# privefl/bigsnpr

Hardware: NVIDIA H100
Metric: genotypes/sec in bed_prodVec (higher is better)
Workload: dtype f64

## Files before the change

### bigsnpr_b200/csrc/bsg_pmv.cu

```cuda
#include <algorithm>
#include <math.h>
#include <stdio.h>
#include <stdlib.h>
#include <string.h>

#include <cub/device/device_scan.cuh>

#include "bsg_internal.cuh"
#include "bsg_pmv_shared.cuh"

namespace bsg {
namespace pmv {

constexpr int SEG = 128;
constexpr int CODES = 512;
constexpr int DIG = 4096;
constexpr int STAGES = 6;
constexpr int STAGE_BYTES = 2 * DIG;
constexpr int SMEM_BYTES = STAGES * STAGE_BYTES + 128;
constexpr int MAX_CHUNKS_PER_ITEM = 512;

struct Args {
  const uint8_t *P;
  int64_t stride;
// ... 532 lines not shown
  int ks_min = (a.nchunks + MAX_CHUNKS_PER_ITEM - 1) / MAX_CHUNKS_PER_ITEM;
  ks = std::min(ks, ks_max);
  ks = std::max(ks, ks_min);
  ks = std::max(ks, 1);
  a.chunks_per_split = (a.nchunks + ks - 1) / ks;
  a.ksplit = (a.nchunks + a.chunks_per_split - 1) / a.chunks_per_split;
  a.dig1 = dig1;
  a.dig2 = dig2;
  a.na_flags = na_flags;
  a.use_na = use_na;
  BSG_TRY(v->s_part.ensure((size_t)a.nlines_pad * 16 * sizeof(long long)));
  a.part = v->s_part.as<long long>();
  BSG_CUDA(cudaMemsetAsync(a.part, 0, (size_t)a.nlines_pad * 16 * sizeof(long long), s));
  const int mode = plane_hi ? 3 : (!use_na ? 0 : (dig2 ? 2 : 1));
  if (plane_hi && !dig2) return fail(BSG_ERR_ARG, "high-bit plane needs its own digits");
  void (*kern)(const Args) = nullptr;
#define PMV_PICK(CWv, Rv, Sv)                                                                   \
  if (var_cw == CWv && var_r == Rv && var_s == Sv)                                              \
    kern = mode == 0 ? k_pmv<0, CWv, Rv, Sv>                                                    \
                     : (mode == 1 ? k_pmv<1, CWv, Rv, Sv> : (mode == 2 ? k_pmv<2, CWv, Rv, Sv> : k_pmv<3, CWv, Rv, Sv>));
  PMV_PICK(11, 2, 0)
  PMV_PICK(11, 2, 1)
  PMV_PICK(11, 2, 2)
  PMV_PICK(11, 3, 0)
  PMV_PICK(11, 3, 1)
  PMV_PICK(15, 2, 1)
#undef PMV_PICK
  if (!kern) return fail(BSG_ERR_ARG, "unknown k_pmv variant");
  BSG_CUDA(cudaFuncSetAttribute(kern, cudaFuncAttributeMaxDynamicSharedMemorySize, SMEM_BYTES));
  int nsm = 132;
  cudaDeviceGetAttribute(&nsm, cudaDevAttrMultiProcessorCount, v->h->device);
  int nitems = ngroups * a.ksplit;
  int grid = std::min(nitems, nsm);
  if (g_timing) cudaEventRecord(g_ev0[g_ev_n % EV_POOL], s);
  kern<<<grid, (var_cw + 1) * 32, SMEM_BYTES, s>>>(a);
  if (g_timing) {
    cudaEventRecord(g_ev1[g_ev_n % EV_POOL], s);
    g_ev_n++;
  }
  count_launch();
  BSG_CUDA(cudaGetLastError());
  *out_args = a;
  return BSG_OK;
}

}

namespace pmvt {
using namespace pmv;
constexpr int TLINES = 32, TBYTES = 512, TWARPS = 8, TSTAGES = 6;
constexpr int WSTAGE_BYTES = TLINES * 64;
constexpr int TSMEM = TWARPS * TSTAGES * WSTAGE_BYTES;
constexpr int MAX_LINES_PER_ITEM = 1 << 16;

struct TArgs {
  const uint8_t *P;
  int64_t stride;
  const int *lines;
  int nlines;
  const uint8_t *dig;
  int lines_per_split, ksplit, nblocks, n;
  long long *part;
};

__device__ __forceinline__ void cp_async16(uint32_t dst, const void *src, int src_bytes) {
  asm volatile("cp.async.cg.shared.global [%0], [%1], 16, %2;" ::"r"(dst), "l"(src), "r"(src_bytes) : "memory");
}

template <int PLANE>
__global__ void __launch_bounds__(TWARPS * 32, 2) k_pmvT_lines(const TArgs a) {
  extern __shared__ __align__(128) uint8_t smem[];
  const int tid = threadIdx.x, warp = tid >> 5, lane = tid & 31, g = lane >> 2, q = lane & 3;
  const int blk = blockIdx.x % a.nblocks, ks = blockIdx.x / a.nblocks;
  const int64_t byte0 = (int64_t)blk * TBYTES + 64 * warp;
  const int l0 = ks * a.lines_per_split, l1 = min(a.nlines, l0 + a.lines_per_split);
  const int nsteps = (l1 - l0 + TLINES - 1) / TLINES;
  const uint32_t wbase = smem_u32(smem) + warp * (TSTAGES * WSTAGE_BYTES);

  const int lrow = lane >> 2, lch = lane & 3;
  const int64_t colb = (byte0 + 16 * lch < a.stride) ? byte0 + 16 * lch : 0;
  uint32_t dst_off[4];
#pragma unroll
  for (int i = 0; i < 4; i++) {
    const int row = 8 * i + lrow;
    const int hf = row >> 4, qq = (row >> 2) & 3, r = row & 3, sl = lch >> 1, hc = lch & 1;
    dst_off[i] = (uint32_t)((((((r * 2 + hf) * 2 + sl) * 4 + qq) * 8) + 4 * hc) * 4);
  }
  auto issue = [&](int step, int stage) {
    const uint32_t dst = wbase + stage * WSTAGE_BYTES;
#pragma unroll
    for (int i = 0; i < 4; i++) {
      const int t = min(l0 + step * TLINES + 8 * i + lrow, l1 - 1);
      const int phys = a.lines[t];
      cp_async16(dst + dst_off[i], a.P + colb + (int64_t)phys * a.stride, 16);
    }
  };

  int acc[4][4][4];
#pragma unroll
  for (int j = 0; j < 4; j++)
#pragma unroll
    for (int c = 0; c < 4; c++)
#pragma unroll
      for (int k = 0; k < 4; k++) acc[j][c][k] = 0;

#pragma unroll
  for (int st = 0; st < TSTAGES - 1; st++) {
    if (st < nsteps) issue(st, st);
    asm volatile("cp.async.commit_group;" ::: "memory");
  }
  const uint8_t *dg = a.dig + (int64_t)(l0 / TLINES) * 256 + g * 32 + 4 * q;
  uint32_t nb0 = 0, nb1 = 0;
  if (nsteps > 0) {
    nb0 = *reinterpret_cast<const uint32_t *>(dg);
    nb1 = *reinterpret_cast<const uint32_t *>(dg + 16);
  }
  const uint32_t rd_base = wbase + (uint32_t)((q * 8 + g) * 4);

  auto compute = [&](uint32_t st_base, uint32_t b0, uint32_t b1) {
    uint32_t W[2][2][4];
// ... 25 lines not shown
        wd = (wd >> 1) & 0x55555555u;
      }
      mma_u8s8(acc[j][0], wa & 0x03030303u, wb & 0x03030303u, wc2 & 0x03030303u, wd & 0x03030303u, b0, b1);
      mma_u8s8(acc[j][1], wa & 0x0C0C0C0Cu, wb & 0x0C0C0C0Cu, wc2 & 0x0C0C0C0Cu, wd & 0x0C0C0C0Cu, b0, b1);
      mma_u8s8(acc[j][2], wa & 0x30303030u, wb & 0x30303030u, wc2 & 0x30303030u, wd & 0x30303030u, b0, b1);
      mma_u8s8(acc[j][3], wa & 0xC0C0C0C0u, wb & 0xC0C0C0C0u, wc2 & 0xC0C0C0C0u, wd & 0xC0C0C0C0u, b0, b1);
    }
  };

  uint32_t rd_stage = 0, wr_stage = (TSTAGES - 1) * WSTAGE_BYTES;
  const uint8_t *dgn = dg + 256;
  for (int step = 0; step < nsteps; step++) {
    asm volatile("cp.async.wait_group %0;" ::"n"(TSTAGES - 2) : "memory");
    __syncwarp();
    {
      const int nxt = step + TSTAGES - 1;
      if (nxt < nsteps) issue(nxt, (int)(wr_stage / WSTAGE_BYTES));
      asm volatile("cp.async.commit_group;" ::: "memory");
    }
    const uint32_t b0 = nb0, b1 = nb1;
    if (step + 1 < nsteps) {
      nb0 = *reinterpret_cast<const uint32_t *>(dgn);
      nb1 = *reinterpret_cast<const uint32_t *>(dgn + 16);
      dgn += 256;
    }
    compute(rd_base + rd_stage, b0, b1);
    rd_stage = rd_stage + WSTAGE_BYTES == TSTAGES * WSTAGE_BYTES ? 0 : rd_stage + WSTAGE_BYTES;
    wr_stage = wr_stage + WSTAGE_BYTES == TSTAGES * WSTAGE_BYTES ? 0 : wr_stage + WSTAGE_BYTES;
  }
  asm volatile("cp.async.wait_group 0;" ::: "memory");
#pragma unroll
  for (int j = 0; j < 4; j++)
#pragma unroll
    for (int c = 0; c < 4; c++)
#pragma unroll
      for (int sl = 0; sl < 2; sl++) {
        const int64_t sample = 4 * (byte0 + 4 * (8 * sl + g) + j) + c;
        if (sample < a.n) {
          unsigned long long *dst = reinterpret_cast<unsigned long long *>(a.part) + sample * 16 + (PLANE ? 8 : 0) + 2 * q;
          long long v0 = acc[j][c][2 * sl], v1 = acc[j][c][2 * sl + 1];
          v0 >>= 2 * c;
          v1 >>= 2 * c;
          if (v0) atomicAdd(dst, (unsigned long long)v0);
          if (v1) atomicAdd(dst + 1, (unsigned long long)v1);
        }
      }
}

constexpr int TBOX = 32 * 128;
constexpr int TDIG_OFF = 4 * TBOX;
constexpr int TSTAGE_BYTES = 4 * TBOX + 1024;
constexpr int TCSTAGES = 6;
constexpr int TSMEM_TMA = TCSTAGES * TSTAGE_BYTES + 2 * TCSTAGES * 8 + 1024;


template <int PLANE>
__global__ void __launch_bounds__(TWARPS * 32, 2) k_pmvT(const __grid_constant__ CUtensorMap map, const TArgs a) {
  extern __shared__ __align__(128) uint8_t smem[];
  const int tid = threadIdx.x, warp = tid >> 5, lane = tid & 31, g = lane >> 2, q = lane & 3;
  const int blk = blockIdx.x % a.nblocks, ks = blockIdx.x / a.nblocks;
  const int l0 = ks * a.lines_per_split, l1 = min(a.nlines, l0 + a.lines_per_split);
  const int nsteps = (l1 - l0 + TLINES - 1) / TLINES;
  const uint32_t sbase = (smem_u32(smem) + 1023u) & ~1023u;
  const uint32_t bar_base = sbase + TCSTAGES * TSTAGE_BYTES;
  auto fill = [&](int step, int st) {
    const uint32_t full = bar_base + 8 * st, dst = sbase + st * TSTAGE_BYTES;
    const uint8_t *dg = a.dig + (int64_t)(l0 / TLINES + step) * 256;
    mbar_expect_tx(full, 4 * TBOX + 256);
#pragma unroll
    for (int j = 0; j < 4; j++) tma_load_2d(dst + j * TBOX, &map, full, blk * TBYTES + 128 * j, l0 + step * TLINES);
    bulk_g2s(dst + TDIG_OFF, dg, 128, full);
    bulk_g2s(dst + TDIG_OFF + 144, dg + 128, 128, full);
  };
  if (tid == 0) {
    for (int st = 0; st < TCSTAGES; st++) {
      mbar_init(bar_base + 8 * st, 1);
      mbar_init(bar_base + 8 * (TCSTAGES + st), TWARPS);
    }
    asm volatile("fence.mbarrier_init.release.cluster;" ::: "memory");
    for (int st = 0; st < min(TCSTAGES, nsteps); st++) fill(st, st);
  }
  __syncthreads();
  int stage = 0, pstage = 0;
  uint32_t phase = 0, pphase = 0;

  const int64_t byte0 = (int64_t)blk * TBYTES + 64 * warp;
  const int rsw = 2 * (q >> 1);
  const uint32_t chunk0 = (4 * (warp & 1) + (g >> 2)) ^ (4 * (q & 1) + rsw);
  const uint32_t rd_base = sbase + (warp >> 1) * TBOX + q * 512 + (rsw << 7) + chunk0 * 16 + 4 * (g & 3);
  const uint32_t dg_base = sbase + TDIG_OFF + g * 32 + 16 * (g >> 2) + 4 * q;
  const uint32_t sel_lo = rsw ? 0x1054u : 0x5410u, sel_hi = rsw ? 0x3276u : 0x7632u;

  int acc[4][4][4];
#pragma unroll
  for (int j = 0; j < 4; j++)
#pragma unroll
    for (int c = 0; c < 4; c++)
#pragma unroll
      for (int k = 0; k < 4; k++) acc[j][c][k] = 0;

  for (int step = 0; step < nsteps; step++) {
    const uint32_t full = bar_base + 8 * stage, empty = bar_base + 8 * (TCSTAGES + stage);
    const uint32_t so = stage * TSTAGE_BYTES;
    const int cstage = stage;
    const uint32_t cphase = phase;
    mbar_wait(full, phase);
    const uint32_t b0 = lds32(dg_base + so), b1 = lds32(dg_base + so + 16);
    uint32_t W[2][2][4];
#pragma unroll
    for (int sl = 0; sl < 2; sl++)
#pragma unroll
      for (int hf = 0; hf < 2; hf++) {
        const uint32_t ad = rd_base + so, hb = hf * (16 * 128);
        const uint32_t x0 = lds32((ad ^ TRD(0, sl)) + hb), x1 = lds32((ad ^ TRD(1, sl)) + hb);
        const uint32_t x2 = lds32((ad ^ TRD(2, sl)) + hb), x3 = lds32((ad ^ TRD(3, sl)) + hb);
        const uint32_t t0 = prmt(x0, x1, 0x5140), t1 = prmt(x2, x3, 0x5140);
        const uint32_t t2 = prmt(x0, x1, 0x7362), t3 = prmt(x2, x3, 0x7362);
        W[sl][hf][0] = prmt(t0, t1, sel_lo);
        W[sl][hf][1] = prmt(t0, t1, sel_hi);
        W[sl][hf][2] = prmt(t2, t3, sel_lo);
        W[sl][hf][3] = prmt(t2, t3, sel_hi);
      }
    __syncwarp();
    if (lane == 0) mbar_arrive(empty);
    if (++stage == TCSTAGES) {
      stage = 0;
      phase ^= 1;
    }
#pragma unroll
    for (int j = 0; j < 4; j++) {
      uint32_t wa = W[0][0][j], wb = W[1][0][j], wc2 = W[0][1][j], wd = W[1][1][j];
      if (PLANE == 1) {
        wa = wa & (wa >> 1) & 0x55555555u;
        wb = wb & (wb >> 1) & 0x55555555u;
        wc2 = wc2 & (wc2 >> 1) & 0x55555555u;
        wd = wd & (wd >> 1) & 0x55555555u;
      } else if (PLANE == 2) {
        wa = (wa >> 1) & 0x55555555u;
        wb = (wb >> 1) & 0x55555555u;
        wc2 = (wc2 >> 1) & 0x55555555u;
        wd = (wd >> 1) & 0x55555555u;
      }
      mma_u8s8(acc[j][0], wa & 0x03030303u, wb & 0x03030303u, wc2 & 0x03030303u, wd & 0x03030303u, b0, b1);
      mma_u8s8(acc[j][1], wa & 0x0C0C0C0Cu, wb & 0x0C0C0C0Cu, wc2 & 0x0C0C0C0Cu, wd & 0x0C0C0C0Cu, b0, b1);
      mma_u8s8(acc[j][2], wa & 0x30303030u, wb & 0x30303030u, wc2 & 0x30303030u, wd & 0x30303030u, b0, b1);
      mma_u8s8(acc[j][3], wa & 0xC0C0C0C0u, wb & 0xC0C0C0C0u, wc2 & 0xC0C0C0C0u, wd & 0xC0C0C0C0u, b0, b1);
    }
    if (tid == 0 && step >= 1 && step - 1 + TCSTAGES < nsteps) {
      mbar_wait(bar_base + 8 * (TCSTAGES + pstage), pphase);
      fill(step - 1 + TCSTAGES, pstage);
    }
    __syncwarp();
    pstage = cstage;
    pphase = cphase;
  }
#pragma unroll
  for (int j = 0; j < 4; j++)
#pragma unroll
    for (int c = 0; c < 4; c++)
#pragma unroll
      for (int sl = 0; sl < 2; sl++) {
        const int64_t sample = 4 * (byte0 + 4 * (8 * sl + g) + j) + c;
        if (sample < a.n) {
          unsigned long long *dst = reinterpret_cast<unsigned long long *>(a.part) + sample * 16 + (PLANE ? 8 : 0) + 2 * q;
          long long v0 = acc[j][c][2 * sl], v1 = acc[j][c][2 * sl + 1];
          v0 >>= 2 * c;
          v1 >>= 2 * c;
          if (v0) atomicAdd(dst, (unsigned long long)v0);
          if (v1) atomicAdd(dst + 1, (unsigned long long)v1);
        }
      }
}

constexpr int W2STAGE_BYTES = TLINES * 32;
constexpr int T2BYTES = TWARPS * 32;
constexpr int T2SMEM = TWARPS * TSTAGES * W2STAGE_BYTES;

template <int PL, bool LINES>
__global__ void __launch_bounds__(TWARPS * 32, 2) k_pmvT2(const TArgs a, const uint8_t *__restrict__ dig2) {
  extern __shared__ __align__(128) uint8_t smem[];
  const int tid = threadIdx.x, warp = tid >> 5, lane = tid & 31, g = lane >> 2, q = lane & 3;
  const int blk = blockIdx.x % a.nblocks, ks = blockIdx.x / a.nblocks;
  const int64_t byte0 = (int64_t)blk * T2BYTES + 32 * warp;
  const int l0 = ks * a.lines_per_split, l1 = min(a.nlines, l0 + a.lines_per_split);
  const int nsteps = (l1 - l0 + TLINES - 1) / TLINES;
  const uint32_t wbase = smem_u32(smem) + warp * (TSTAGES * W2STAGE_BYTES);
  const int lrow = lane >> 1, lch = lane & 1;
  const int64_t colb = (byte0 + 16 * lch < a.stride) ? byte0 + 16 * lch : 0;
  uint32_t dst_off[2];
#pragma unroll
  for (int i = 0; i < 2; i++) {
    const int row = 16 * i + lrow;
    const int hf = row >> 4, qq = (row >> 2) & 3, r = row & 3;
    dst_off[i] = (uint32_t)(((((r * 2 + hf) * 4 + qq) * 8) + 4 * lch) * 4);
  }
  const int full_steps = (l1 - l0) / TLINES;
  const int64_t stride16 = 16 * a.stride;
  auto issue = [&](int step, int stage) {
    const uint32_t dst = wbase + stage * W2STAGE_BYTES;
#pragma unroll
    for (int i = 0; i < 2; i++) {
      const int t = min(l0 + step * TLINES + 16 * i + lrow, l1 - 1);
      const int phys = LINES ? a.lines[t] : t;
      cp_async16(dst + dst_off[i], a.P + colb + (int64_t)phys * a.stride, 16);
    }
  };
  int acc[2][2][4][4];
#pragma unroll
  for (int p = 0; p < 2; p++)
#pragma unroll
    for (int u = 0; u < 2; u++)
#pragma unroll
      for (int c = 0; c < 4; c++)
#pragma unroll
        for (int k = 0; k < 4; k++) acc[p][u][c][k] = 0;
#pragma unroll
  for (int st = 0; st < TSTAGES - 1; st++) {
    if (st < nsteps) issue(st, st);
    asm volatile("cp.async.commit_group;" ::: "memory");
  }
  const int64_t doff = (int64_t)(l0 / TLINES) * 256 + g * 32 + 4 * q;
  const uint8_t *dg = a.dig + doff, *dp = dig2 + doff;
  uint32_t nb0 = 0, nb1 = 0, np0 = 0, np1 = 0;
  if (nsteps > 0) {
// ... 332 lines not shown
  using namespace pmvt;
  bsg_bed *h = v->h;
  const int n = h->n, nc = v->nc;
  const int nsteps = (nc + TLINES - 1) / TLINES;
  BSG_TRY(v->s_part.ensure((size_t)std::max(n, 1) * 16 * sizeof(long long)));
  long long *part = v->s_part.as<long long>();
  *part_out = part;
  BSG_CUDA(cudaMemsetAsync(part, 0, (size_t)n * 16 * sizeof(long long), s));
  if (nc == 0 || n == 0) return BSG_OK;
  TArgs a;
  a.P = h->A;
  a.stride = h->strideA;
  a.lines = v->d_col;
  a.nlines = nc;
  a.n = n;
  a.part = part;
  const int64_t nbytes = ((int64_t)n + 3) / 4;
  a.nblocks = (int)((nbytes + TBYTES - 1) / TBYTES);
  int nsm = 132;
  cudaDeviceGetAttribute(&nsm, cudaDevAttrMultiProcessorCount, h->device);
  static int waves = 0;
  if (!waves) {
    const char *ev = getenv("BSG_PMVT_WAVES");
    waves = ev ? std::max(1, std::min(64, atoi(ev))) : 4;
  }
  auto pick_ks = [&](int nblocks) {
    const int slots = 2 * nsm;
    const int lo = std::max(1, (nc + MAX_LINES_PER_ITEM - 1) / MAX_LINES_PER_ITEM);
    const int hi = std::max(lo, std::min(std::max(1, nsteps / 32), std::max(lo, (4 * waves * slots) / std::max(nblocks, 1))));
    static int force_ks = -1;
    if (force_ks < 0) {
      const char *ev = getenv("BSG_PMVT_KS");
      force_ks = ev ? std::max(0, atoi(ev)) : 0;
    }
    if (force_ks > 0) return std::max(lo, force_ks);
    int best = lo;
    double best_score = -1;
    for (int ks = lo; ks <= hi; ks++) {
      const double ctas = (double)nblocks * ks, nwav = ceil(ctas / slots);
      double score = ctas / (nwav * slots);
      const double lines = (double)nc / ks;
      score *= lines / (lines + 1000.0);
      if (nwav < waves) score *= 0.9 + 0.1 * nwav / waves;
      if (score > best_score + 1e-9) {
        best_score = score;
        best = ks;
      }
    }
    return best;
  };
  int ks = pick_ks(a.nblocks);
  a.lines_per_split = (int)round_up((nc + ks - 1) / ks, TLINES);
  a.ksplit = (nc + a.lines_per_split - 1) / a.lines_per_split;
  static unsigned attr_done = 0;
  if (!(attr_done >> (h->device & 31) & 1u)) {
    BSG_CUDA(cudaFuncSetAttribute(k_pmvT<0>, cudaFuncAttributeMaxDynamicSharedMemorySize, TSMEM_TMA));
    BSG_CUDA(cudaFuncSetAttribute(k_pmvT_lines<0>, cudaFuncAttributeMaxDynamicSharedMemorySize, TSMEM));
    BSG_CUDA(cudaFuncSetAttribute(k_pmvT2<1, false>, cudaFuncAttributeMaxDynamicSharedMemorySize, T2SMEM));
    BSG_CUDA(cudaFuncSetAttribute(k_pmvT2<1, true>, cudaFuncAttributeMaxDynamicSharedMemorySize, T2SMEM));
    BSG_CUDA(cudaFuncSetAttribute(k_pmvT2<2, false>, cudaFuncAttributeMaxDynamicSharedMemorySize, T2SMEM));
    BSG_CUDA(cudaFuncSetAttribute(k_pmvT2<2, true>, cudaFuncAttributeMaxDynamicSharedMemorySize, T2SMEM));
    attr_done |= 1u << (h->device & 31);
  }
  const int thr = TWARPS * 32;
  const bool lines = a.lines != nullptr;
  a.dig = dig_raw;
  if (g_timing) cudaEventRecord(g_ev0[g_ev_n % EV_POOL], s);
  if (!plane) {
    const int grid = a.nblocks * a.ksplit;
    if (lines) {
      k_pmvT_lines<0><<<grid, thr, TSMEM, s>>>(a);
    } else {
      CUtensorMap map;
      BSG_TRY(make_map(&map, a.P, nc, a.stride, TLINES));
      k_pmvT<0><<<grid, thr, TSMEM_TMA, s>>>(map, a);
    }
  } else {
    a.nblocks = (int)((nbytes + T2BYTES - 1) / T2BYTES);
    const int ks2 = pick_ks(a.nblocks);
    a.lines_per_split = (int)round_up((nc + ks2 - 1) / ks2, TLINES);
    a.ksplit = (nc + a.lines_per_split - 1) / a.lines_per_split;
    const int grid = a.nblocks * a.ksplit;
    if (plane == 1) {
      if (lines)
        k_pmvT2<1, true><<<grid, thr, T2SMEM, s>>>(a, dig_plane);
      else
        k_pmvT2<1, false><<<grid, thr, T2SMEM, s>>>(a, dig_plane);
    } else {
      if (lines)
        k_pmvT2<2, true><<<grid, thr, T2SMEM, s>>>(a, dig_plane);
      else
        k_pmvT2<2, false><<<grid, thr, T2SMEM, s>>>(a, dig_plane);
    }
  }
  if (g_timing) {
    cudaEventRecord(g_ev1[g_ev_n % EV_POOL], s);
    g_ev_n++;
  }
  count_launch();
  BSG_CUDA(cudaGetLastError());
  return BSG_OK;
}

static int prep_T(bsg_view *v, int mode, const double *x, const double *p1, const double *p2, int nv, const double *xb,
                  bool two, cudaStream_t s, long long *qna_full = nullptr, int na_second = 0) {
  using namespace pmv;
  using namespace pmvt;
  Scal *sc = v->s_scal.as<Scal>();
  const int nc = v->nc;
  const int nsteps = (nc + TLINES - 1) / TLINES;
  BSG_TRY(v->s_dig1.ensure((size_t)std::max(nsteps, 1) * 256));
  if (two) BSG_TRY(v->s_dig2.ensure((size_t)std::max(nsteps, 1) * 256));
  uint8_t *dig1 = v->s_dig1.as<uint8_t>(), *dig2 = two ? v->s_dig2.as<uint8_t>() : nullptr;
  BSG_CUDA(cudaMemsetAsync(sc, 0, nv * sizeof(Scal), s));
  k_prep1<<<SUMCZ_BLOCKS, 256, 0, s>>>(mode, x, p1, p2, nc, 0, sc);
  if (xb) k_prep1<<<SUMCZ_BLOCKS, 256, 0, s>>>(mode, xb, p1, p2, nc, 0, sc + 1);
  const int grid = launch_cap((int64_t)std::max(nsteps, 1) * TLINES, 256, 1184);
  if (nv == 1)
    k_quantT<1><<<grid, 256, 0, s>>>(mode, x, nullptr, p1, p2, nc, nsteps * TLINES, sc, dig1, dig2, v->d_col, qna_full,
                                     na_second);
  else
    k_quantT<2><<<grid, 256, 0, s>>>(mode, x, xb, p1, p2, nc, nsteps * TLINES, sc, dig1, dig2, nullptr, nullptr, 0);
  count_launch(xb ? 3 : 2);
  return BSG_OK;
}

static int prodvec_T(bsg_view *v, const double *x_dev, double *out_dev, cudaStream_t s, bsg_comm *comm) {
  using namespace pmv;
  bsg_bed *h = v->h;
  Scal *sc = v->s_scal.as<Scal>();
  const int n = h->n, nc = v->nc;
  const int mode = v->has_scaling ? 1 : 0;
  const bool lists = h->has_na && na_ell_ready(h);
  const bool two = v->has_scaling && h->has_na && !lists;
// ... 778 lines not shown
```

### bigsnpr_b200/csrc/bsg_pmv_shared.cuh

```cuda
#pragma once
#include <cuda.h>
#include <math.h>
#include <stdint.h>

namespace bsg {
namespace pmv {

constexpr int SUMCZ_BLOCKS = 128;

__device__ __forceinline__ uint32_t smem_u32(const void *p) { return (uint32_t)__cvta_generic_to_shared(p); }

__device__ __forceinline__ void mbar_init(uint32_t bar, uint32_t count) {
  asm volatile("mbarrier.init.shared::cta.b64 [%0], %1;" ::"r"(bar), "r"(count));
}
__device__ __forceinline__ void mbar_expect_tx(uint32_t bar, uint32_t bytes) {
  asm volatile("mbarrier.arrive.expect_tx.shared::cta.b64 _, [%0], %1;" ::"r"(bar), "r"(bytes) : "memory");
}
__device__ __forceinline__ void mbar_arrive(uint32_t bar) {
  asm volatile("mbarrier.arrive.shared::cta.b64 _, [%0];" ::"r"(bar) : "memory");
}
__device__ __forceinline__ void mbar_wait(uint32_t bar, uint32_t parity) {
  asm volatile(
      "{\n\t.reg .pred p;\n\t"
      "WAIT_%=:\n\t"
      "mbarrier.try_wait.parity.shared::cta.b64 p, [%0], %1;\n\t"
      "@p bra DONE_%=;\n\t"
      "bra WAIT_%=;\n\t"
      "DONE_%=:\n\t}" ::"r"(bar),
      "r"(parity)
      : "memory");
}
__device__ __forceinline__ void bulk_g2s(uint32_t dst, const void *src, uint32_t bytes, uint32_t bar) {
  asm volatile("cp.async.bulk.shared::cluster.global.mbarrier::complete_tx::bytes [%0], [%1], %2, [%3];" ::"r"(dst),
               "l"(src), "r"(bytes), "r"(bar)
               : "memory");
}
__device__ __forceinline__ void mma_u8s8(int (&d)[4], uint32_t a0, uint32_t a1, uint32_t a2, uint32_t a3,
                                         uint32_t b0, uint32_t b1) {
  asm volatile(
      "mma.sync.aligned.m16n8k32.row.col.s32.u8.s8.s32 {%0,%1,%2,%3}, {%4,%5,%6,%7}, {%8,%9}, {%0,%1,%2,%3};"
      : "+r"(d[0]), "+r"(d[1]), "+r"(d[2]), "+r"(d[3])
      : "r"(a0), "r"(a1), "r"(a2), "r"(a3), "r"(b0), "r"(b1));
}
__device__ __forceinline__ uint4 lds128(uint32_t addr) {
  uint4 v;
  asm volatile("ld.shared.v4.u32 {%0,%1,%2,%3}, [%4];" : "=r"(v.x), "=r"(v.y), "=r"(v.z), "=r"(v.w) : "r"(addr));
  return v;
}

__device__ __forceinline__ uint4 ldg_stream(const uint8_t *p) {
  uint4 v;
  asm volatile("ld.global.nc.L1::no_allocate.v4.u32 {%0,%1,%2,%3}, [%4];"
               : "=r"(v.x), "=r"(v.y), "=r"(v.z), "=r"(v.w)
               : "l"(p));
  return v;
}

__device__ __forceinline__ uint32_t lds32(uint32_t addr) {
  uint32_t v;
  asm volatile("ld.shared.u32 %0, [%1];" : "=r"(v) : "r"(addr));
  return v;
}
__device__ __forceinline__ uint32_t prmt(uint32_t a, uint32_t b, uint32_t sel) {
  uint32_t r;
  asm("prmt.b32 %0, %1, %2, %3;" : "=r"(r) : "r"(a), "r"(b), "r"(sel));
  return r;
}

__device__ __forceinline__ void tma_load_2d(uint32_t dst, const CUtensorMap *map, uint32_t bar, int c0, int c1) {
  asm volatile(
      "cp.async.bulk.tensor.2d.shared::cluster.global.mbarrier::complete_tx::bytes [%0], [%1, {%3, %4}], [%2];" ::"r"(dst),
      "l"(map), "r"(bar), "r"(c0), "r"(c1)
      : "memory");
}

__host__ __device__ constexpr uint32_t TRD(int i, int sl) { return (uint32_t)((i << 7) ^ (i << 4) ^ (sl << 5)); }

__device__ __forceinline__ int pick_e(double m, int hb, int bits) {
  int ex = 0;
  if (m > 0 && isfinite(m)) {
    frexp(m, &ex);
    return bits - ex - hb;
  }
  return 0;
}

__device__ __forceinline__ int peel(long long &q) {
  const int d = (int)(signed char)(q & 0xFF);
  q = (q - d) >> 8;
  return d;
}

struct Scal {
  double maxabs[2];
  int nonfinite;
  int e[2];
  int hb;
  long long sum_hi, sum_lo;
  double cpart[128];
};

template <int NS>
__device__ __forceinline__ double combine(const long long *__restrict__ part, int64_t line, int s0, int c0, int c1, int e) {
  const long long *p = part + line * 16 + s0;
  double acc = 0;
#pragma unroll
  for (int s = NS - 1; s >= 0; s--) {
    long long v = 0;
    if (c0) v += c0 * p[s];
    if (c1) v += c1 * p[8 + s];
    acc += scalbn((double)v, 8 * s - e);
  }
  return acc;
// ... 19 lines not shown
```

Before: 12030 billion.

## Load genotype tiles with ldmatrix.trans and use cumulative masks for code planes

Replaces the 16 scalar shared-memory loads and 12 byte permutes per step with four ldmatrix x4 transposed loads plus 8 permutes, and rearranges the digit B-fragment loads to match the new lane-to-sample mapping. The per-code MMA masks become cumulative (low 2, 4, 6, 8 bits), which saves mask instructions, and the per-code partial sums are recovered by differencing adjacent accumulators before writing out. A fake data dependence (a xor of the loaded values ANDed with a sign bit that is always zero) is added to the empty-barrier arrive so the loads complete before the stage is released. This cuts instruction count in the inner loop but relies on the new sample mapping and the accumulator differences being exactly right, and cumulative masks make the later accumulators hold larger values.

```diff
diff --git a/bigsnpr_b200/csrc/bsg_pmv.cu b/bigsnpr_b200/csrc/bsg_pmv.cu
--- a/bigsnpr_b200/csrc/bsg_pmv.cu
+++ b/bigsnpr_b200/csrc/bsg_pmv.cu
@@ -786,11 +786,9 @@
   uint32_t phase = 0, pphase = 0;
 
   const int64_t byte0 = (int64_t)blk * TBYTES + 64 * warp;
-  const int rsw = 2 * (q >> 1);
-  const uint32_t chunk0 = (4 * (warp & 1) + (g >> 2)) ^ (4 * (q & 1) + rsw);
-  const uint32_t rd_base = sbase + (warp >> 1) * TBOX + q * 512 + (rsw << 7) + chunk0 * 16 + 4 * (g & 3);
-  const uint32_t dg_base = sbase + TDIG_OFF + g * 32 + 16 * (g >> 2) + 4 * q;
-  const uint32_t sel_lo = rsw ? 0x1054u : 0x5410u, sel_hi = rsw ? 0x3276u : 0x7632u;
+  const uint32_t rd_base = sbase + (warp >> 1) * TBOX + lane * 128 + 16 * ((4 * (warp & 1)) ^ (lane & 7));
+  const uint32_t dg_base = sbase + TDIG_OFF + g * 32 + 16 * (g >> 2) + 4 * (q >> 1);
+  const uint32_t bsel = (q & 1) ? 0x7632u : 0x5410u;
 
   int acc[4][4][4];
 #pragma unroll
@@ -806,31 +804,28 @@
     const int cstage = stage;
     const uint32_t cphase = phase;
     mbar_wait(full, phase);
-    const uint32_t b0 = lds32(dg_base + so), b1 = lds32(dg_base + so + 16);
-    uint32_t W[2][2][4];
-#pragma unroll
-    for (int sl = 0; sl < 2; sl++)
-#pragma unroll
-      for (int hf = 0; hf < 2; hf++) {
-        const uint32_t ad = rd_base + so, hb = hf * (16 * 128);
-        const uint32_t x0 = lds32((ad ^ TRD(0, sl)) + hb), x1 = lds32((ad ^ TRD(1, sl)) + hb);
-        const uint32_t x2 = lds32((ad ^ TRD(2, sl)) + hb), x3 = lds32((ad ^ TRD(3, sl)) + hb);
-        const uint32_t t0 = prmt(x0, x1, 0x5140), t1 = prmt(x2, x3, 0x5140);
-        const uint32_t t2 = prmt(x0, x1, 0x7362), t3 = prmt(x2, x3, 0x7362);
-        W[sl][hf][0] = prmt(t0, t1, sel_lo);
-        W[sl][hf][1] = prmt(t0, t1, sel_hi);
-        W[sl][hf][2] = prmt(t2, t3, sel_lo);
-        W[sl][hf][3] = prmt(t2, t3, sel_hi);
-      }
+    const uint32_t d0 = lds32(dg_base + so), d1 = lds32(dg_base + so + 8);
+    const uint32_t d2 = lds32(dg_base + so + 16), d3 = lds32(dg_base + so + 24);
+    uint32_t A[4][4];
+#pragma unroll
+    for (int j = 0; j < 4; j++) {
+      const uint4 R = ldsm_x4_trans((rd_base + so) ^ (j << 4));
+      A[j][0] = prmt(R.x, R.y, 0x6420);
+      A[j][1] = prmt(R.x, R.y, 0x7531);
+      A[j][2] = prmt(R.z, R.w, 0x6420);
+      A[j][3] = prmt(R.z, R.w, 0x7531);
+    }
+    const uint32_t b0 = prmt(d0, d1, bsel), b1 = prmt(d2, d3, bsel);
+    const uint32_t landed = (A[0][0] ^ A[1][0] ^ A[2][0] ^ A[3][0] ^ b0 ^ b1) & ((uint32_t)a.nblocks >> 31);
     __syncwarp();
-    if (lane == 0) mbar_arrive(empty);
+    if (lane == 0) mbar_arrive(empty + landed);
     if (++stage == TCSTAGES) {
       stage = 0;
       phase ^= 1;
     }
 #pragma unroll
     for (int j = 0; j < 4; j++) {
-      uint32_t wa = W[0][0][j], wb = W[1][0][j], wc2 = W[0][1][j], wd = W[1][1][j];
+      uint32_t wa = A[j][0], wb = A[j][1], wc2 = A[j][2], wd = A[j][3];
       if (PLANE == 1) {
         wa = wa & (wa >> 1) & 0x55555555u;
         wb = wb & (wb >> 1) & 0x55555555u;
@@ -843,9 +838,9 @@
         wd = (wd >> 1) & 0x55555555u;
       }
       mma_u8s8(acc[j][0], wa & 0x03030303u, wb & 0x03030303u, wc2 & 0x03030303u, wd & 0x03030303u, b0, b1);
-      mma_u8s8(acc[j][1], wa & 0x0C0C0C0Cu, wb & 0x0C0C0C0Cu, wc2 & 0x0C0C0C0Cu, wd & 0x0C0C0C0Cu, b0, b1);
-      mma_u8s8(acc[j][2], wa & 0x30303030u, wb & 0x30303030u, wc2 & 0x30303030u, wd & 0x30303030u, b0, b1);
-      mma_u8s8(acc[j][3], wa & 0xC0C0C0C0u, wb & 0xC0C0C0C0u, wc2 & 0xC0C0C0C0u, wd & 0xC0C0C0C0u, b0, b1);
+      mma_u8s8(acc[j][1], wa & 0x0F0F0F0Fu, wb & 0x0F0F0F0Fu, wc2 & 0x0F0F0F0Fu, wd & 0x0F0F0F0Fu, b0, b1);
+      mma_u8s8(acc[j][2], wa & 0x3F3F3F3Fu, wb & 0x3F3F3F3Fu, wc2 & 0x3F3F3F3Fu, wd & 0x3F3F3F3Fu, b0, b1);
+      mma_u8s8(acc[j][3], wa, wb, wc2, wd, b0, b1);
     }
     if (tid == 0 && step >= 1 && step - 1 + TCSTAGES < nsteps) {
       mbar_wait(bar_base + 8 * (TCSTAGES + pstage), pphase);
@@ -860,11 +855,15 @@
 #pragma unroll
     for (int c = 0; c < 4; c++)
 #pragma unroll
-      for (int sl = 0; sl < 2; sl++) {
-        const int64_t sample = 4 * (byte0 + 4 * (8 * sl + g) + j) + c;
+      for (int hi = 0; hi < 2; hi++) {
+        const int64_t sample = 4 * (byte0 + 16 * j + 2 * g + hi) + c;
         if (sample < a.n) {
           unsigned long long *dst = reinterpret_cast<unsigned long long *>(a.part) + sample * 16 + (PLANE ? 8 : 0) + 2 * q;
-          long long v0 = acc[j][c][2 * sl], v1 = acc[j][c][2 * sl + 1];
+          long long v0 = acc[j][c][2 * hi], v1 = acc[j][c][2 * hi + 1];
+          if (c) {
+            v0 -= acc[j][c - 1][2 * hi];
+            v1 -= acc[j][c - 1][2 * hi + 1];
+          }
           v0 >>= 2 * c;
           v1 >>= 2 * c;
           if (v0) atomicAdd(dst, (unsigned long long)v0);
diff --git a/bigsnpr_b200/csrc/bsg_pmv_shared.cuh b/bigsnpr_b200/csrc/bsg_pmv_shared.cuh
--- a/bigsnpr_b200/csrc/bsg_pmv_shared.cuh
+++ b/bigsnpr_b200/csrc/bsg_pmv_shared.cuh
@@ -59,6 +59,13 @@
 __device__ __forceinline__ uint32_t lds32(uint32_t addr) {
   uint32_t v;
   asm volatile("ld.shared.u32 %0, [%1];" : "=r"(v) : "r"(addr));
+  return v;
+}
+__device__ __forceinline__ uint4 ldsm_x4_trans(uint32_t addr) {
+  uint4 v;
+  asm volatile("ldmatrix.sync.aligned.m8n8.x4.trans.shared.b16 {%0,%1,%2,%3}, [%4];"
+               : "=r"(v.x), "=r"(v.y), "=r"(v.z), "=r"(v.w)
+               : "r"(addr));
   return v;
 }
 __device__ __forceinline__ uint32_t prmt(uint32_t a, uint32_t b, uint32_t sel) {
```

Result: faster. 12170 billion, median of 6 (+1.2%).

## Use ldmatrix.trans loads, cumulative masks, and rotating-warp TMA producer in k_pmvT

Applied to the files above, without the earlier changes.

Replaces the sixteen per-thread 32-bit shared loads and two-level byte permutes with four ldmatrix.x4.trans loads followed by a single permute level. The per-code masks become cumulative (low 2, 4, 6, 8 bits), so the last MMA takes raw words and the masking ALU work shrinks; adjacent accumulators are differenced at the end to recover each 2-bit field. The loop is unrolled over the stage ring, empty barriers now count all threads, and the refill role rotates across warps using elect.sync instead of being fixed to thread 0. The cumulative masks enlarge MMA operand values, so a static_assert guards int32 accumulator overflow, and the per-thread arrive adds barrier traffic.

```diff
diff --git a/bigsnpr_b200/csrc/bsg_pmv.cu b/bigsnpr_b200/csrc/bsg_pmv.cu
--- a/bigsnpr_b200/csrc/bsg_pmv.cu
+++ b/bigsnpr_b200/csrc/bsg_pmv.cu
@@ -608,6 +608,7 @@
 constexpr int WSTAGE_BYTES = TLINES * 64;
 constexpr int TSMEM = TWARPS * TSTAGES * WSTAGE_BYTES;
 constexpr int MAX_LINES_PER_ITEM = 1 << 16;
+static_assert(255LL * 128 * MAX_LINES_PER_ITEM < (1LL << 31), "k_pmvT accumulators would overflow");
 
 struct TArgs {
   const uint8_t *P;
@@ -753,118 +754,132 @@
 constexpr int TSTAGE_BYTES = 4 * TBOX + 1024;
 constexpr int TCSTAGES = 6;
 constexpr int TSMEM_TMA = TCSTAGES * TSTAGE_BYTES + 2 * TCSTAGES * 8 + 1024;
-
+constexpr unsigned long long TLDSM_ROWS = 0xfe985432dcba7610ull;
+
+__device__ __forceinline__ void ldsm_x4_trans(uint32_t addr, uint32_t (&r)[4]) {
+  asm volatile("ldmatrix.sync.aligned.m8n8.x4.trans.shared.b16 {%0,%1,%2,%3}, [%4];"
+               : "=r"(r[0]), "=r"(r[1]), "=r"(r[2]), "=r"(r[3])
+               : "r"(addr));
+}
+__device__ __forceinline__ bool elect_one() {
+  uint32_t p;
+  asm volatile("{\n\t.reg .pred P;\n\telect.sync _|P, 0xffffffff;\n\tselp.u32 %0, 1, 0, P;\n\t}" : "=r"(p));
+  return p != 0;
+}
 
 template <int PLANE>
 __global__ void __launch_bounds__(TWARPS * 32, 2) k_pmvT(const __grid_constant__ CUtensorMap map, const TArgs a) {
   extern __shared__ __align__(128) uint8_t smem[];
-  const int tid = threadIdx.x, warp = tid >> 5, lane = tid & 31, g = lane >> 2, q = lane & 3;
+  const int tid = threadIdx.x, lane = tid & 31, g = lane >> 2, q = lane & 3;
+  const int warp = __shfl_sync(0xffffffffu, tid >> 5, 0);
   const int blk = blockIdx.x % a.nblocks, ks = blockIdx.x / a.nblocks;
   const int l0 = ks * a.lines_per_split, l1 = min(a.nlines, l0 + a.lines_per_split);
   const int nsteps = (l1 - l0 + TLINES - 1) / TLINES;
   const uint32_t sbase = (smem_u32(smem) + 1023u) & ~1023u;
   const uint32_t bar_base = sbase + TCSTAGES * TSTAGE_BYTES;
   auto fill = [&](int step, int st) {
-    const uint32_t full = bar_base + 8 * st, dst = sbase + st * TSTAGE_BYTES;
-    const uint8_t *dg = a.dig + (int64_t)(l0 / TLINES + step) * 256;
-    mbar_expect_tx(full, 4 * TBOX + 256);
-#pragma unroll
-    for (int j = 0; j < 4; j++) tma_load_2d(dst + j * TBOX, &map, full, blk * TBYTES + 128 * j, l0 + step * TLINES);
-    bulk_g2s(dst + TDIG_OFF, dg, 128, full);
-    bulk_g2s(dst + TDIG_OFF + 144, dg + 128, 128, full);
+    if (elect_one()) {
+      const uint32_t full = bar_base + 8 * st, dst = sbase + st * TSTAGE_BYTES;
+      const uint8_t *dg = a.dig + (int64_t)(l0 / TLINES + step) * 256;
+      mbar_expect_tx(full, 4 * TBOX + 256);
+#pragma unroll
+      for (int j = 0; j < 4; j++) tma_load_2d(dst + j * TBOX, &map, full, blk * TBYTES + 128 * j, l0 + step * TLINES);
+      bulk_g2s(dst + TDIG_OFF, dg, 128, full);
+      bulk_g2s(dst + TDIG_OFF + 144, dg + 128, 128, full);
+    }
   };
-  if (tid == 0) {
+  if (warp == 0) {
+    if (elect_one()) {
+      for (int st = 0; st < TCSTAGES; st++) {
+        mbar_init(bar_base + 8 * st, 1);
+        mbar_init(bar_base + 8 * (TCSTAGES + st), TWARPS * 32);
+      }
+      asm volatile("fence.mbarrier_init.release.cluster;" ::: "memory");
+    }
+    __syncwarp();
+    for (int st = 0; st < min(TCSTAGES, nsteps); st++) fill(st, st);
+  }
+  __syncthreads();
+
+  const int64_t byte0 = (int64_t)blk * TBYTES + 64 * warp;
+  const int m = lane >> 3;
+  const int line = (int)((TLDSM_ROWS >> (4 * (8 * (m & 1) + (lane & 7)))) & 15) + 16 * (m >> 1);
+  const uint32_t rd0 = sbase + (warp >> 1) * TBOX + line * 128 + (((4 * (warp & 1)) ^ (line & 7)) << 4);
+  uint32_t rd[4];
+#pragma unroll
+  for (int j = 0; j < 4; j++) rd[j] = rd0 ^ (j << 4);
+  const uint32_t dg_base = sbase + TDIG_OFF + g * 32 + 16 * (g >> 2) + 4 * q;
+  const bool xlo = q == 0 || q == 3;
+  const uint32_t sel_lo = xlo ? 0x6420u : 0x2064u, sel_hi = xlo ? 0x7531u : 0x3175u;
+
+  int acc[4][4][4];
+#pragma unroll
+  for (int j = 0; j < 4; j++)
+#pragma unroll
+    for (int c = 0; c < 4; c++)
+#pragma unroll
+      for (int k = 0; k < 4; k++) acc[j][c][k] = 0;
+
+  uint32_t phase = 0;
+  for (int base = 0; base < nsteps; base += TCSTAGES, phase ^= 1) {
+#pragma unroll
     for (int st = 0; st < TCSTAGES; st++) {
-      mbar_init(bar_base + 8 * st, 1);
-      mbar_init(bar_base + 8 * (TCSTAGES + st), TWARPS);
-    }
-    asm volatile("fence.mbarrier_init.release.cluster;" ::: "memory");
-    for (int st = 0; st < min(TCSTAGES, nsteps); st++) fill(st, st);
-  }
-  __syncthreads();
-  int stage = 0, pstage = 0;
-  uint32_t phase = 0, pphase = 0;
-
-  const int64_t byte0 = (int64_t)blk * TBYTES + 64 * warp;
-  const int rsw = 2 * (q >> 1);
-  const uint32_t chunk0 = (4 * (warp & 1) + (g >> 2)) ^ (4 * (q & 1) + rsw);
-  const uint32_t rd_base = sbase + (warp >> 1) * TBOX + q * 512 + (rsw << 7) + chunk0 * 16 + 4 * (g & 3);
-  const uint32_t dg_base = sbase + TDIG_OFF + g * 32 + 16 * (g >> 2) + 4 * q;
-  const uint32_t sel_lo = rsw ? 0x1054u : 0x5410u, sel_hi = rsw ? 0x3276u : 0x7632u;
-
-  int acc[4][4][4];
+      const int step = base + st;
+      if (step >= nsteps) break;
+      const uint32_t so = st * TSTAGE_BYTES;
+      mbar_wait(bar_base + 8 * st, phase);
+      const uint32_t b0 = lds32(dg_base + so), b1 = lds32(dg_base + so + 16);
+      uint32_t W[4][4];
+#pragma unroll
+      for (int j = 0; j < 4; j++) {
+        uint32_t r[4];
+        ldsm_x4_trans(rd[j] + so, r);
+        W[j][0] = prmt(r[0], r[1], sel_lo);
+        W[j][1] = prmt(r[0], r[1], sel_hi);
+        W[j][2] = prmt(r[2], r[3], sel_lo);
+        W[j][3] = prmt(r[2], r[3], sel_hi);
+      }
+#pragma unroll
+      for (int j = 0; j < 4; j++) {
+        uint32_t wa = W[j][0], wb = W[j][1], wc2 = W[j][2], wd = W[j][3];
+        if (PLANE == 1) {
+          wa = wa & (wa >> 1) & 0x55555555u;
+          wb = wb & (wb >> 1) & 0x55555555u;
+          wc2 = wc2 & (wc2 >> 1) & 0x55555555u;
+          wd = wd & (wd >> 1) & 0x55555555u;
+        } else if (PLANE == 2) {
+          wa = (wa >> 1) & 0x55555555u;
+          wb = (wb >> 1) & 0x55555555u;
+          wc2 = (wc2 >> 1) & 0x55555555u;
+          wd = (wd >> 1) & 0x55555555u;
+        }
+        mma_u8s8(acc[j][0], wa & 0x03030303u, wb & 0x03030303u, wc2 & 0x03030303u, wd & 0x03030303u, b0, b1);
+        mma_u8s8(acc[j][1], wa & 0x0F0F0F0Fu, wb & 0x0F0F0F0Fu, wc2 & 0x0F0F0F0Fu, wd & 0x0F0F0F0Fu, b0, b1);
+        mma_u8s8(acc[j][2], wa & 0x3F3F3F3Fu, wb & 0x3F3F3F3Fu, wc2 & 0x3F3F3F3Fu, wd & 0x3F3F3F3Fu, b0, b1);
+        mma_u8s8(acc[j][3], wa, wb, wc2, wd, b0, b1);
+      }
+      if (warp == (step & (TWARPS - 1)) && step >= 1 && step - 1 + TCSTAGES < nsteps) {
+        const int pst = st ? st - 1 : TCSTAGES - 1;
+        mbar_wait(bar_base + 8 * (TCSTAGES + pst), st ? phase : phase ^ 1);
+        fill(step - 1 + TCSTAGES, pst);
+      }
+      mbar_arrive(bar_base + 8 * (TCSTAGES + st));
+    }
+  }
 #pragma unroll
   for (int j = 0; j < 4; j++)
 #pragma unroll
     for (int c = 0; c < 4; c++)
 #pragma unroll
-      for (int k = 0; k < 4; k++) acc[j][c][k] = 0;
-
-  for (int step = 0; step < nsteps; step++) {
-    const uint32_t full = bar_base + 8 * stage, empty = bar_base + 8 * (TCSTAGES + stage);
-    const uint32_t so = stage * TSTAGE_BYTES;
-    const int cstage = stage;
-    const uint32_t cphase = phase;
-    mbar_wait(full, phase);
-    const uint32_t b0 = lds32(dg_base + so), b1 = lds32(dg_base + so + 16);
-    uint32_t W[2][2][4];
-#pragma unroll
-    for (int sl = 0; sl < 2; sl++)
-#pragma unroll
-      for (int hf = 0; hf < 2; hf++) {
-        const uint32_t ad = rd_base + so, hb = hf * (16 * 128);
-        const uint32_t x0 = lds32((ad ^ TRD(0, sl)) + hb), x1 = lds32((ad ^ TRD(1, sl)) + hb);
-        const uint32_t x2 = lds32((ad ^ TRD(2, sl)) + hb), x3 = lds32((ad ^ TRD(3, sl)) + hb);
-        const uint32_t t0 = prmt(x0, x1, 0x5140), t1 = prmt(x2, x3, 0x5140);
-        const uint32_t t2 = prmt(x0, x1, 0x7362), t3 = prmt(x2, x3, 0x7362);
-        W[sl][hf][0] = prmt(t0, t1, sel_lo);
-        W[sl][hf][1] = prmt(t0, t1, sel_hi);
-        W[sl][hf][2] = prmt(t2, t3, sel_lo);
-        W[sl][hf][3] = prmt(t2, t3, sel_hi);
-      }
-    __syncwarp();
-    if (lane == 0) mbar_arrive(empty);
-    if (++stage == TCSTAGES) {
-      stage = 0;
-      phase ^= 1;
-    }
-#pragma unroll
-    for (int j = 0; j < 4; j++) {
-      uint32_t wa = W[0][0][j], wb = W[1][0][j], wc2 = W[0][1][j], wd = W[1][1][j];
-      if (PLANE == 1) {
-        wa = wa & (wa >> 1) & 0x55555555u;
-        wb = wb & (wb >> 1) & 0x55555555u;
-        wc2 = wc2 & (wc2 >> 1) & 0x55555555u;
-        wd = wd & (wd >> 1) & 0x55555555u;
-      } else if (PLANE == 2) {
-        wa = (wa >> 1) & 0x55555555u;
-        wb = (wb >> 1) & 0x55555555u;
-        wc2 = (wc2 >> 1) & 0x55555555u;
-        wd = (wd >> 1) & 0x55555555u;
-      }
-      mma_u8s8(acc[j][0], wa & 0x03030303u, wb & 0x03030303u, wc2 & 0x03030303u, wd & 0x03030303u, b0, b1);
-      mma_u8s8(acc[j][1], wa & 0x0C0C0C0Cu, wb & 0x0C0C0C0Cu, wc2 & 0x0C0C0C0Cu, wd & 0x0C0C0C0Cu, b0, b1);
-      mma_u8s8(acc[j][2], wa & 0x30303030u, wb & 0x30303030u, wc2 & 0x30303030u, wd & 0x30303030u, b0, b1);
-      mma_u8s8(acc[j][3], wa & 0xC0C0C0C0u, wb & 0xC0C0C0C0u, wc2 & 0xC0C0C0C0u, wd & 0xC0C0C0C0u, b0, b1);
-    }
-    if (tid == 0 && step >= 1 && step - 1 + TCSTAGES < nsteps) {
-      mbar_wait(bar_base + 8 * (TCSTAGES + pstage), pphase);
-      fill(step - 1 + TCSTAGES, pstage);
-    }
-    __syncwarp();
-    pstage = cstage;
-    pphase = cphase;
-  }
-#pragma unroll
-  for (int j = 0; j < 4; j++)
-#pragma unroll
-    for (int c = 0; c < 4; c++)
-#pragma unroll
-      for (int sl = 0; sl < 2; sl++) {
-        const int64_t sample = 4 * (byte0 + 4 * (8 * sl + g) + j) + c;
+      for (int e = 0; e < 2; e++) {
+        const int64_t sample = 4 * (byte0 + 16 * j + 2 * g + e) + c;
         if (sample < a.n) {
           unsigned long long *dst = reinterpret_cast<unsigned long long *>(a.part) + sample * 16 + (PLANE ? 8 : 0) + 2 * q;
-          long long v0 = acc[j][c][2 * sl], v1 = acc[j][c][2 * sl + 1];
+          long long v0 = acc[j][c][2 * e], v1 = acc[j][c][2 * e + 1];
+          if (c) {
+            v0 -= acc[j][c - 1][2 * e];
+            v1 -= acc[j][c - 1][2 * e + 1];
+          }
           v0 >>= 2 * c;
           v1 >>= 2 * c;
           if (v0) atomicAdd(dst, (unsigned long long)v0);
```

Result: faster. 12030 billion before, 12280 billion after (median of 6 runs) (+2.1%).

## Use ldmatrix.trans for transposed genotype loads and cumulative masks in TMA pmvT

Applied to the files above, without the earlier changes.

The TMA transposed product kernel now fetches its genotype tiles with ldmatrix x4 transposed loads and a smaller set of byte permutes, replacing per-lane 32-bit shared loads and a deeper prmt shuffle. The per-code masks become cumulative (low 2, 4, 6, 8 bits), so the last MMA uses raw words, and the epilogue recovers each code by subtracting the previous accumulator. The empty-barrier arrive moves to the start of the next iteration, which removes a syncwarp. The cumulative sums need more int32 headroom, so a guard now rejects k-splits longer than a fixed line count.

```diff
diff --git a/bigsnpr_b200/csrc/bsg_pmv.cu b/bigsnpr_b200/csrc/bsg_pmv.cu
--- a/bigsnpr_b200/csrc/bsg_pmv.cu
+++ b/bigsnpr_b200/csrc/bsg_pmv.cu
@@ -622,6 +622,15 @@
 __device__ __forceinline__ void cp_async16(uint32_t dst, const void *src, int src_bytes) {
   asm volatile("cp.async.cg.shared.global [%0], [%1], 16, %2;" ::"r"(dst), "l"(src), "r"(src_bytes) : "memory");
 }
+__device__ __forceinline__ void ldsm_x4_trans(uint32_t (&r)[4], uint32_t addr) {
+  asm volatile("ldmatrix.sync.aligned.m8n8.x4.trans.shared.b16 {%0,%1,%2,%3}, [%4];"
+               : "=r"(r[0]), "=r"(r[1]), "=r"(r[2]), "=r"(r[3])
+               : "r"(addr));
+}
+__device__ __forceinline__ uint32_t pin(uint32_t v) {
+  asm volatile("mov.b32 %0, %0;" : "+r"(v));
+  return v;
+}
 
 template <int PLANE>
 __global__ void __launch_bounds__(TWARPS * 32, 2) k_pmvT_lines(const TArgs a) {
@@ -786,11 +795,15 @@
   uint32_t phase = 0, pphase = 0;
 
   const int64_t byte0 = (int64_t)blk * TBYTES + 64 * warp;
-  const int rsw = 2 * (q >> 1);
-  const uint32_t chunk0 = (4 * (warp & 1) + (g >> 2)) ^ (4 * (q & 1) + rsw);
-  const uint32_t rd_base = sbase + (warp >> 1) * TBOX + q * 512 + (rsw << 7) + chunk0 * 16 + 4 * (g & 3);
-  const uint32_t dg_base = sbase + TDIG_OFF + g * 32 + 16 * (g >> 2) + 4 * q;
-  const uint32_t sel_lo = rsw ? 0x1054u : 0x5410u, sel_hi = rsw ? 0x3276u : 0x7632u;
+  const int mi = lane >> 3, mr = lane & 7;
+  const int mline = 4 * (mr >> 1) + (mr & 1) + 2 * ((mr >> 2) ^ (mi & 1));
+  auto rd_addr = [&](int u) {
+    const int chunk = (4 * (warp & 1) + 2 * u + (mi >> 1)) ^ (mline & 7);
+    return sbase + (warp >> 1) * TBOX + mline * 128 + chunk * 16;
+  };
+  const uint32_t rd0 = pin(rd_addr(0)), rd1 = pin(rd_addr(1));
+  const uint32_t dg_base = pin(sbase + TDIG_OFF + g * 32 + 16 * (g >> 2) + 4 * q);
+  const uint32_t sel_ev = pin(q >= 2 ? 0x2064u : 0x6420u), sel_od = pin(q >= 2 ? 0x3175u : 0x7531u);
 
   int acc[4][4][4];
 #pragma unroll
@@ -801,36 +814,34 @@
       for (int k = 0; k < 4; k++) acc[j][c][k] = 0;
 
   for (int step = 0; step < nsteps; step++) {
-    const uint32_t full = bar_base + 8 * stage, empty = bar_base + 8 * (TCSTAGES + stage);
+    const uint32_t full = bar_base + 8 * stage;
     const uint32_t so = stage * TSTAGE_BYTES;
     const int cstage = stage;
     const uint32_t cphase = phase;
+    if (step > 0 && lane == 0) mbar_arrive(bar_base + 8 * (TCSTAGES + pstage));
     mbar_wait(full, phase);
     const uint32_t b0 = lds32(dg_base + so), b1 = lds32(dg_base + so + 16);
-    uint32_t W[2][2][4];
-#pragma unroll
-    for (int sl = 0; sl < 2; sl++)
+    uint32_t R[2][2][4];
+#pragma unroll
+    for (int u = 0; u < 2; u++)
+#pragma unroll
+      for (int hf = 0; hf < 2; hf++) ldsm_x4_trans(R[u][hf], (u ? rd1 : rd0) + so + hf * (16 * 128));
+    uint32_t W[4][2][2];
+#pragma unroll
+    for (int ch = 0; ch < 4; ch++)
 #pragma unroll
       for (int hf = 0; hf < 2; hf++) {
-        const uint32_t ad = rd_base + so, hb = hf * (16 * 128);
-        const uint32_t x0 = lds32((ad ^ TRD(0, sl)) + hb), x1 = lds32((ad ^ TRD(1, sl)) + hb);
-        const uint32_t x2 = lds32((ad ^ TRD(2, sl)) + hb), x3 = lds32((ad ^ TRD(3, sl)) + hb);
-        const uint32_t t0 = prmt(x0, x1, 0x5140), t1 = prmt(x2, x3, 0x5140);
-        const uint32_t t2 = prmt(x0, x1, 0x7362), t3 = prmt(x2, x3, 0x7362);
-        W[sl][hf][0] = prmt(t0, t1, sel_lo);
-        W[sl][hf][1] = prmt(t0, t1, sel_hi);
-        W[sl][hf][2] = prmt(t2, t3, sel_lo);
-        W[sl][hf][3] = prmt(t2, t3, sel_hi);
+        const uint32_t x = R[ch >> 1][hf][2 * (ch & 1)], y = R[ch >> 1][hf][2 * (ch & 1) + 1];
+        W[ch][hf][0] = prmt(x, y, sel_ev);
+        W[ch][hf][1] = prmt(x, y, sel_od);
       }
-    __syncwarp();
-    if (lane == 0) mbar_arrive(empty);
     if (++stage == TCSTAGES) {
       stage = 0;
       phase ^= 1;
     }
 #pragma unroll
     for (int j = 0; j < 4; j++) {
-      uint32_t wa = W[0][0][j], wb = W[1][0][j], wc2 = W[0][1][j], wd = W[1][1][j];
+      uint32_t wa = W[j & 2][0][j & 1], wb = W[(j & 2) + 1][0][j & 1], wc2 = W[j & 2][1][j & 1], wd = W[(j & 2) + 1][1][j & 1];
       if (PLANE == 1) {
         wa = wa & (wa >> 1) & 0x55555555u;
         wb = wb & (wb >> 1) & 0x55555555u;
@@ -843,9 +854,9 @@
         wd = (wd >> 1) & 0x55555555u;
       }
       mma_u8s8(acc[j][0], wa & 0x03030303u, wb & 0x03030303u, wc2 & 0x03030303u, wd & 0x03030303u, b0, b1);
-      mma_u8s8(acc[j][1], wa & 0x0C0C0C0Cu, wb & 0x0C0C0C0Cu, wc2 & 0x0C0C0C0Cu, wd & 0x0C0C0C0Cu, b0, b1);
-      mma_u8s8(acc[j][2], wa & 0x30303030u, wb & 0x30303030u, wc2 & 0x30303030u, wd & 0x30303030u, b0, b1);
-      mma_u8s8(acc[j][3], wa & 0xC0C0C0C0u, wb & 0xC0C0C0C0u, wc2 & 0xC0C0C0C0u, wd & 0xC0C0C0C0u, b0, b1);
+      mma_u8s8(acc[j][1], wa & 0x0F0F0F0Fu, wb & 0x0F0F0F0Fu, wc2 & 0x0F0F0F0Fu, wd & 0x0F0F0F0Fu, b0, b1);
+      mma_u8s8(acc[j][2], wa & 0x3F3F3F3Fu, wb & 0x3F3F3F3Fu, wc2 & 0x3F3F3F3Fu, wd & 0x3F3F3F3Fu, b0, b1);
+      mma_u8s8(acc[j][3], wa, wb, wc2, wd, b0, b1);
     }
     if (tid == 0 && step >= 1 && step - 1 + TCSTAGES < nsteps) {
       mbar_wait(bar_base + 8 * (TCSTAGES + pstage), pphase);
@@ -858,19 +869,25 @@
 #pragma unroll
   for (int j = 0; j < 4; j++)
 #pragma unroll
-    for (int c = 0; c < 4; c++)
-#pragma unroll
-      for (int sl = 0; sl < 2; sl++) {
-        const int64_t sample = 4 * (byte0 + 4 * (8 * sl + g) + j) + c;
+    for (int sl = 0; sl < 2; sl++) {
+      const int64_t sbyte = byte0 + 16 * ((j & 2) + sl) + 2 * g + (j & 1);
+#pragma unroll
+      for (int c = 0; c < 4; c++) {
+        const int64_t sample = 4 * sbyte + c;
         if (sample < a.n) {
           unsigned long long *dst = reinterpret_cast<unsigned long long *>(a.part) + sample * 16 + (PLANE ? 8 : 0) + 2 * q;
           long long v0 = acc[j][c][2 * sl], v1 = acc[j][c][2 * sl + 1];
+          if (c) {
+            v0 -= acc[j][c - 1][2 * sl];
+            v1 -= acc[j][c - 1][2 * sl + 1];
+          }
           v0 >>= 2 * c;
           v1 >>= 2 * c;
           if (v0) atomicAdd(dst, (unsigned long long)v0);
           if (v1) atomicAdd(dst + 1, (unsigned long long)v1);
         }
       }
+    }
 }
 
 constexpr int W2STAGE_BYTES = TLINES * 32;
@@ -1309,6 +1326,7 @@
   int ks = pick_ks(a.nblocks);
   a.lines_per_split = (int)round_up((nc + ks - 1) / ks, TLINES);
   a.ksplit = (nc + a.lines_per_split - 1) / a.lines_per_split;
+  if (a.lines_per_split > MAX_LINES_PER_ITEM) return fail(BSG_ERR_ARG, "k-split of %d lines exceeds the int32 head-room", a.lines_per_split);
   static unsigned attr_done = 0;
   if (!(attr_done >> (h->device & 31) & 1u)) {
     BSG_CUDA(cudaFuncSetAttribute(k_pmvT<0>, cudaFuncAttributeMaxDynamicSharedMemorySize, TSMEM_TMA));
@@ -1337,6 +1355,7 @@
     const int ks2 = pick_ks(a.nblocks);
     a.lines_per_split = (int)round_up((nc + ks2 - 1) / ks2, TLINES);
     a.ksplit = (nc + a.lines_per_split - 1) / a.lines_per_split;
+    if (a.lines_per_split > MAX_LINES_PER_ITEM) return fail(BSG_ERR_ARG, "k-split of %d lines exceeds the int32 head-room", a.lines_per_split);
     const int grid = a.nblocks * a.ksplit;
     if (plane == 1) {
       if (lines)
```

Result: no change. 12030 billion before, 12120 billion after (median of 6 runs) (+0.8%).
